# lijingzhu1/SKGHOI

Hardware: AMD Instinct MI355X
Metric: images/sec through interaction head (20x20 pairs) (higher is better)
Workload: dtype f32; 1 GPU; HICO-DET-shaped synthetic cached detections: 20 humans x 20 objects per image (G=800 grid rows, P=780 pairs, K=117 verbs), eval forward of InteractionHead from cached AdaMixer-R50 box features [40,256,7,7]/image; precision=fp32, batch_per_gpu=256, parallelism=dp1 (independent image shards, no data-path collective)

## Files before the change

### skghoi_amd/csrc/skg_gemm.hip

```cpp
#include "skg_common.h"
#include <string.h>
#include <atomic>
#include <type_traits>

__device__ __forceinline__ float skg_exp2i(int e) { return __uint_as_float((uint32_t)(127 + e) << 23); }

typedef _Float16 f16x8 __attribute__((ext_vector_type(8)));
typedef _Float16 h16x2 __attribute__((ext_vector_type(2)));
typedef uint32_t u32x4 __attribute__((ext_vector_type(4)));
typedef short s16x8 __attribute__((ext_vector_type(8)));
typedef __bf16 bf16x2_t __attribute__((ext_vector_type(2)));
typedef float f32x2_t __attribute__((ext_vector_type(2)));

__device__ __forceinline__ uint32_t skg_pack_bf16x2(float a, float b) {
    const f32x2_t v = {a, b};
    return __builtin_bit_cast(uint32_t, __builtin_convertvector(v, bf16x2_t));
}
__device__ __forceinline__ void skg_store_bf16x4(uint16_t* p, float a, float b, float c, float e) {
    *reinterpret_cast<uint2*>(p) = make_uint2(skg_pack_bf16x2(a, b), skg_pack_bf16x2(c, e));
}
__device__ __forceinline__ void skg_store_bf16(uint16_t* p, float a) { *p = (uint16_t)(skg_pack_bf16x2(a, 0.f) & 0xffffu); }

#define BM 128
#define BN 128
// ... 1048 lines not shown
struct skg_gemm_group_args {
    skg_gemm_desc d[SKG_GEMM_GROUP_MAX];
    int start[SKG_GEMM_GROUP_MAX + 1];
    int n;
};

__global__ __launch_bounds__(256, SKG_MINW) void skg_gemm_group_kernel(const skg_gemm_group_args g) {
    __shared__ __attribute__((aligned(16))) float smem[2 * (A_TILE + B_TILE)];
    int k = 0;
#pragma unroll
    for (int t = 1; t < SKG_GEMM_GROUP_MAX; ++t)
        if (t < g.n && (int)blockIdx.x >= g.start[t]) k = t;
    skg_gemm_tile<-1, 0, 2>(g.d[k], blockIdx.x - g.start[k], smem);
}

__global__ __launch_bounds__(256, SKG_MINW) void skg_gemm_group_split_kernel(const skg_gemm_group_args g) {
    __shared__ __attribute__((aligned(16))) float smem[2 * (A_TILE + B_TILE)];
    int k = 0;
#pragma unroll
    for (int t = 1; t < SKG_GEMM_GROUP_MAX; ++t)
        if (t < g.n && (int)blockIdx.x >= g.start[t]) k = t;
    skg_gemm_tile<-1, 2, 2>(g.d[k], blockIdx.x - g.start[k], smem);
}

__global__ __launch_bounds__(256, SKG_MINW) void skg_gemm_group_small_kernel(const skg_gemm_group_args g) {
    __shared__ __attribute__((aligned(16))) float smem[4 * 32 * 36];
    int k = 0;
#pragma unroll
    for (int t = 1; t < SKG_GEMM_GROUP_MAX; ++t)
        if (t < g.n && (int)blockIdx.x >= g.start[t]) k = t;
    skg_gemm_tile<-1, 1, 1>(g.d[k], blockIdx.x - g.start[k], smem);
}

__global__ __launch_bounds__(256, SKG_NB4 > 2 ? 1 : SKG_MINW) void skg_gemm_group_direct_kernel(const skg_gemm_group_args g) {
    __shared__ __attribute__((aligned(1024))) float smem[SKG_SMEM4];
    int k = 0;
#pragma unroll
    for (int t = 1; t < SKG_GEMM_GROUP_MAX; ++t)
        if (t < g.n && (int)blockIdx.x >= g.start[t]) k = t;
    skg_gemm_tile<-1, 4, 1>(g.d[k], blockIdx.x - g.start[k], smem);
}

__global__ __launch_bounds__(256, SKG_MINW) void skg_gemm_group_latency_kernel(const skg_gemm_group_args g) {
    __shared__ __attribute__((aligned(16))) float smem[SKG_SMEM3];
    int k = 0;
#pragma unroll
    for (int t = 1; t < SKG_GEMM_GROUP_MAX; ++t)
        if (t < g.n && (int)blockIdx.x >= g.start[t]) k = t;
    skg_gemm_tile<-1, 3, 1>(g.d[k], blockIdx.x - g.start[k], smem);
}

__global__ __launch_bounds__(512, 1) void skg_gemm_group_khalves_kernel(const skg_gemm_group_args g) {
    __shared__ __attribute__((aligned(16))) float smem[SKG_SMEM3];
    int k = 0;
#pragma unroll
    for (int t = 1; t < SKG_GEMM_GROUP_MAX; ++t)
        if (t < g.n && (int)blockIdx.x >= g.start[t]) k = t;
    skg_gemm_tile<-1, 5, 1>(g.d[k], blockIdx.x - g.start[k], smem);
}

#define SKG_SMEM6(T) (2 * 2 * 64 * (T) * 32)
template <int EPI, int T>
__global__ __launch_bounds__(256, 2) void skg_gemm_b16_kernel(const skg_gemm_desc d, const uint16_t* w16) {
    __shared__ __attribute__((aligned(1024))) float smem[SKG_SMEM6(T)];
    skg_gemm_tile<EPI, 6, T>(d, blockIdx.x, smem, w16);
}
// ... 107 lines not shown
    const int src = a_rows ? a_rows[row] : row;
    uint32_t mx = 0u;
    if (src >= 0) {
        const float* p = A + (int64_t)src * lda;
        for (int k = 4 * lane; k < K; k += 256) {
            const float4 v = *reinterpret_cast<const float4*>(p + k);
            mx = max(max(mx, __float_as_uint(v.x) & 0x7fffffffu), __float_as_uint(v.y) & 0x7fffffffu);
            mx = max(max(mx, __float_as_uint(v.z) & 0x7fffffffu), __float_as_uint(v.w) & 0x7fffffffu);
        }
    }
#pragma unroll
    for (int off = 32; off > 0; off >>= 1) mx = max(mx, (uint32_t)__shfl_xor((int)mx, off, 64));
    if (lane == 0) {
        const int E = (int)(mx >> 23);
        exp_out[row] = (mx == 0u || E == 255) ? 0 : min(max(E - 127 - 11, -126), 126);
    }
}

extern "C" int skg_row_exponents_f32(const float* A, int64_t lda, const int32_t* a_rows, int M, int K, int32_t* exp_out,
                                     void* stream) {
    if (M < 0 || K <= 0 || (K & 3) || (lda & 3)) return SKG_E_ARG;
    if (M == 0) return 0;
    if (!A || !exp_out) return SKG_E_ARG;
    if (!skg_aligned16(A)) return SKG_E_ALIGN;
    hipLaunchKernelGGL(skg_row_exponents_kernel, dim3((M + 3) / 4), dim3(256), 0, (hipStream_t)stream, A, lda, a_rows, M, K,
                       exp_out);
    return skg_launch_status();
}

#define g_small_mode skg_tune_small_mode()
#define g_khalves_blocks skg_tune_khalves_blocks()
#define g_small_tiles skg_tune_small_tiles()

static int skg_gemm_tile_scale(const skg_gemm_desc* d) {
    const bool glds = SKG_USE_GLDS && BK == 16 && (d->K % BK) == 0 && !d->a_rows &&
                      (int64_t)BM * d->lda * 4 < 0xffffffffLL && (int64_t)BN * d->ldw * 4 < 0xffffffffLL;
    const int64_t tiles128 = (int64_t)((d->M + 127) / 128) * ((d->N + 127) / 128) * (d->split_k > 1 ? d->split_k : 1);
    if (d->w_split && (d->K % 16) == 0 && d->w_scale > 0.f) return 2;
    return (glds && (tiles128 < g_small_tiles || d->M <= 64)) ? 1 : 2;
}

extern "C" int skg_gemm_dot_partials(const skg_gemm_desc* dh) {
    if (!dh) return SKG_E_ARG;
    const int T = skg_gemm_tile_scale(dh);
    return 2 * ((dh->N + 64 * T - 1) / (64 * T));
}

static int skg_gemm_validate(const skg_gemm_desc& d) {
    if (d.split_k > 1 && (!d.split_ws || (d.epilogue != SKG_EPI_BIAS && d.epilogue != SKG_EPI_BIAS_RELU &&
                                          d.epilogue != SKG_EPI_BIAS_RES_RELU) || d.split_k > 64))
        return SKG_E_ARG;
    if (d.M < 0 || d.N <= 0 || d.K <= 0 || !d.A || !d.W) return SKG_E_ARG;
    if ((d.K & 3) || (d.lda & 3) || (d.ldw & 3)) return SKG_E_ALIGN;
    if (!skg_aligned16(d.A) || !skg_aligned16(d.W)) return SKG_E_ALIGN;
    if (d.lda < d.K && !d.a_rows && d.M > 1) return SKG_E_ARG;
    switch (d.epilogue) {
        case SKG_EPI_BIAS: case SKG_EPI_BIAS_RELU:
            if (!d.C) return SKG_E_ARG; break;
        case SKG_EPI_MUL_RELU:
            if (!d.C || (!d.P && !d.Q)) return SKG_E_ARG; break;
        case SKG_EPI_RELU_DOT:
            if (!d.dot_w || !d.dot_partial) return SKG_E_ARG; break;
        case SKG_EPI_BIAS_RES_RELU:
            if (!d.C || !d.res) return SKG_E_ARG; break;
        default: return SKG_E_ARG;
    }
    return 0;
}

#define g_route_tiles skg_tune_route_tiles()

static bool skg_route_desc(const skg_gemm_desc& d, skg_gemmx_desc& x, skg_gemmx_fused& f) {
    if (d.w_split || d.a_rows || d.a_exp || d.epilogue == SKG_EPI_RELU_DOT) return false;
    memset(&x, 0, sizeof(x)); memset(&f, 0, sizeof(f));
    x.A = d.A; x.a_sm = d.lda; x.a_sk = 1;
    x.B = d.W; x.b_sn = d.ldw; x.b_sk = 1;
    x.C = d.C; x.ldc = d.ldc; x.M = d.M; x.N = d.N; x.K = d.K;
    x.bias = d.bias; x.relu = d.epilogue == SKG_EPI_BIAS_RELU ? 1 : 0;
    x.split_k = d.split_k > 1 ? d.split_k : 0; x.split_ws = d.split_ws;
    f.out_rows = d.out_rows;
    if (d.epilogue == SKG_EPI_MUL_RELU) {
        f.kind = SKG_EPI_MUL_RELU;
        f.P = d.P; f.p_idx = d.p_idx; f.ldp = d.ldp; f.Q = d.Q; f.q_idx = d.q_idx; f.ldq = d.ldq; f.mbias = d.mbias;
        f.C_raw = d.C_raw; f.ldc_raw = d.ldc_raw;
    } else if (d.epilogue == SKG_EPI_BIAS_RES_RELU) {
        f.kind = SKG_EPI_BIAS_RES_RELU; f.res = d.res; f.ldres = d.ldres;
    }
    return skg_gemmx_can_fuse(&x, &f) != 0;
}

static bool skg_gemm_group_small(const skg_gemm_desc* descs, int n) {
    int64_t tiles128 = 0;
    for (int i = 0; i < n; ++i) {
        const skg_gemm_desc& d = descs[i];
        if (d.M == 0) continue;
        const bool glds = SKG_USE_GLDS && BK == 16 && (d.K % BK) == 0 && !d.a_rows &&
                          (int64_t)BM * d.lda * 4 < 0xffffffffLL && (int64_t)BN * d.ldw * 4 < 0xffffffffLL;
        if (!glds || (d.w_split && d.w_scale > 0.f)) return false;
        tiles128 += (int64_t)((d.M + 127) / 128) * ((d.N + 127) / 128);
    }
    return tiles128 < g_small_tiles;
}

static std::atomic<long long> g_gemm_path[SKG_GEMM_PATHS];
static inline void skg_gemm_count(int path) { g_gemm_path[path].fetch_add(1, std::memory_order_relaxed); }

extern "C" void skg_gemm_path_counts(int64_t* out_host, int reset) {
    for (int i = 0; i < SKG_GEMM_PATHS; ++i) {
        if (out_host) out_host[i] = g_gemm_path[i].load(std::memory_order_relaxed);
        if (reset) g_gemm_path[i].store(0, std::memory_order_relaxed);
    }
}

extern "C" int skg_gemm_group_tile(const skg_gemm_desc* descs_host, int n) {
    if (!descs_host || n < 1 || n > SKG_GEMM_GROUP_MAX) return SKG_E_ARG;
    return skg_gemm_group_small(descs_host, n) ? 1 : 2;
}

extern "C" int skg_gemm_group_f32(const skg_gemm_desc* descs_host, int n, void* stream) {
    if (!descs_host || n < 1 || n > SKG_GEMM_GROUP_MAX) return SKG_E_ARG;
    skg_gemm_group_args g, r;
    g.n = r.n = 0;
    int64_t blocks = 0, rblocks = 0;
    bool split = true;
    for (int i = 0; i < n; ++i) {
        const int rc = skg_gemm_validate(descs_host[i]);
        if (rc) return rc;
    }
    const bool small = skg_gemm_group_small(descs_host, n);
    if (n <= SKG_GEMMX_GROUP_MAX) {
// ... 4 lines not shown
        for (int i = 0; i < n && ok; ++i) {
            const skg_gemm_desc& d = descs_host[i];
            ok = skg_route_desc(d, xs[i], fs[i]);
            tiles128 += (int64_t)((d.M + 127) / 128) * ((d.N + 127) / 128) * (d.split_k > 1 ? d.split_k : 1);
        }
        if (ok && tiles128 >= g_route_tiles && tiles128 < 4 * g_small_tiles) {
            skg_gemm_count(SKG_GEMM_PATH_ROUTED);
            return skg_gemmx_f32_fused(xs, fs, n, stream);
        }
    }
    for (int i = 0; i < n; ++i) {
        const skg_gemm_desc& d = descs_host[i];
        if (d.split_k > 1 && !small) return SKG_E_ARG;
        if (d.M == 0) continue;
        split = split && d.w_split && (d.K % 16) == 0 && d.w_scale > 0.f;
        const int64_t nb = skg_gemm_blocks(d.M, d.N, d.K, small ? 1 : 2) * (d.split_k > 1 ? d.split_k : 1);
        if (blocks + nb > 0x7fffffffLL) return SKG_E_LIMIT;
        g.d[g.n] = d;
        g.start[g.n] = (int)blocks;
        blocks += nb;
        ++g.n;
        if (d.split_k > 1) {
            r.d[r.n] = d;
            r.start[r.n] = (int)rblocks;
            rblocks += ((int64_t)d.M * d.N + 255) / 256;
            ++r.n;
        }
    }
    if (g.n == 0) return 0;
    for (int i = g.n; i <= SKG_GEMM_GROUP_MAX; ++i) g.start[i] = (int)blocks;
    bool direct = small && g_small_mode == 4;
    for (int i = 0; i < g.n && direct; ++i) direct = (g.d[i].K % 64) == 0;
    const bool halves = small && (g_small_mode == 5 || (g_small_mode == 6 && blocks <= g_khalves_blocks));
    skg_gemm_count(split && !small ? SKG_GEMM_PATH_FP16X2 : SKG_GEMM_PATH_EXACT);
    if (direct) hipLaunchKernelGGL(skg_gemm_group_direct_kernel, dim3((unsigned)blocks), dim3(256), 0, (hipStream_t)stream, g);
    else if (halves) hipLaunchKernelGGL(skg_gemm_group_khalves_kernel, dim3((unsigned)blocks), dim3(512), 0, (hipStream_t)stream, g);
    else if (small && g_small_mode >= 3) hipLaunchKernelGGL(skg_gemm_group_latency_kernel, dim3((unsigned)blocks), dim3(256), 0, (hipStream_t)stream, g);
    else if (small) hipLaunchKernelGGL(skg_gemm_group_small_kernel, dim3((unsigned)blocks), dim3(256), 0, (hipStream_t)stream, g);
    else if (split) hipLaunchKernelGGL(skg_gemm_group_split_kernel, dim3((unsigned)blocks), dim3(256), 0, (hipStream_t)stream, g);
    else hipLaunchKernelGGL(skg_gemm_group_kernel, dim3((unsigned)blocks), dim3(256), 0, (hipStream_t)stream, g);
    if (r.n) {
        for (int i = r.n; i <= SKG_GEMM_GROUP_MAX; ++i) r.start[i] = (int)rblocks;
        hipLaunchKernelGGL(skg_splitk_reduce_group_kernel, dim3((unsigned)rblocks), dim3(256), 0, (hipStream_t)stream, r);
    }
    return skg_launch_status();
}

extern "C" int skg_gemm_f32(const skg_gemm_desc* dh, void* stream) {
    if (!dh) return SKG_E_ARG;
    const skg_gemm_desc d = *dh;
    const int rc = skg_gemm_validate(d);
    if (rc) return rc;
    if (d.M == 0) return 0;
    const bool glds = SKG_USE_GLDS && BK == 16 && (d.K % BK) == 0 && !d.a_rows &&
                      (int64_t)BM * d.lda * 4 < 0xffffffffLL && (int64_t)BN * d.ldw * 4 < 0xffffffffLL;
    const bool split = d.w_split && (d.K % 16) == 0 && d.w_scale > 0.f;
    const int T = split ? 2 : skg_gemm_tile_scale(&d);
    if (!split && T == 1 && d.M > 64) {
        const int64_t tiles128 = (int64_t)((d.M + 127) / 128) * ((d.N + 127) / 128) * (d.split_k > 1 ? d.split_k : 1);
        skg_gemmx_desc x; skg_gemmx_fused f;
        if (tiles128 >= g_route_tiles && skg_route_desc(d, x, f)) {
            skg_gemm_count(SKG_GEMM_PATH_ROUTED);
            return skg_gemmx_f32_fused(&x, &f, 1, stream);
        }
    }
    const int64_t nblk = skg_gemm_blocks(d.M, d.N, d.K, T) * (d.split_k > 1 ? d.split_k : 1);
    if (nblk > 0x7fffffffLL) return SKG_E_LIMIT;
    dim3 grid((unsigned)nblk), block(256);
    hipStream_t s = (hipStream_t)stream;
    skg_gemm_count(split ? SKG_GEMM_PATH_FP16X2 : SKG_GEMM_PATH_EXACT);
#define SKG_LAUNCH(E)                                                                              \
    if (split) hipLaunchKernelGGL((skg_gemm_kernel<E, 2, 2>), grid, block, 0, s, d);               \
    else if (glds && T == 1 && g_small_mode == 4 && (d.K % 64) == 0) hipLaunchKernelGGL((skg_gemm_kernel<E, 4, 1>), grid, block, 0, s, d); \
    else if (glds && T == 1 && (g_small_mode == 5 || (g_small_mode == 6 && nblk <= g_khalves_blocks))) hipLaunchKernelGGL((skg_gemm_kernel<E, 5, 1>), grid, dim3(512), 0, s, d); \
    else if (glds && T == 1 && g_small_mode >= 3) hipLaunchKernelGGL((skg_gemm_kernel<E, 3, 1>), grid, block, 0, s, d); \
    else if (glds && T == 1) hipLaunchKernelGGL((skg_gemm_kernel<E, 1, 1>), grid, block, 0, s, d); \
    else if (glds) hipLaunchKernelGGL((skg_gemm_kernel<E, 1, 2>), grid, block, 0, s, d);           \
    else hipLaunchKernelGGL((skg_gemm_kernel<E, 0, 2>), grid, block, 0, s, d);
    switch (d.epilogue) {
        case SKG_EPI_BIAS:          SKG_LAUNCH(SKG_EPI_BIAS) break;
        case SKG_EPI_BIAS_RELU:     SKG_LAUNCH(SKG_EPI_BIAS_RELU) break;
        case SKG_EPI_MUL_RELU:      SKG_LAUNCH(SKG_EPI_MUL_RELU) break;
        case SKG_EPI_RELU_DOT:      SKG_LAUNCH(SKG_EPI_RELU_DOT) break;
        case SKG_EPI_BIAS_RES_RELU: SKG_LAUNCH(SKG_EPI_BIAS_RES_RELU) break;
    }
#undef SKG_LAUNCH
    if (d.split_k > 1) {
        const int64_t total = (int64_t)d.M * d.N;
// ... 302 lines not shown
```

### skghoi_amd/csrc/skg_pairs.hip

```cpp
#include "skg_common.h"

#define PS_THREADS 256
__global__ __launch_bounds__(PS_THREADS) void skg_pairs_spatial_kernel(
    const float* __restrict__ boxes, const skg_image_meta* __restrict__ meta, int32_t* __restrict__ grid_h,
    int32_t* __restrict__ grid_o, int32_t* __restrict__ grid_pair, int32_t* __restrict__ grid_img,
    int32_t* __restrict__ pair_grid, int64_t* __restrict__ x_keep, int64_t* __restrict__ y_keep,
    int32_t* __restrict__ pair_h, int32_t* __restrict__ pair_o, float* __restrict__ spatial, int scrub_nan,
    int grid_cap, int pair_cap) {
    __shared__ float4 sbox[SKG_MAX_NODES];
    const int a = blockIdx.x;
    const skg_image_meta mt = meta[a];
    const int lane = threadIdx.x;
    const int n = mt.n, n_h = mt.n_h;
    for (int t = lane; t < n; t += PS_THREADS)
        sbox[t] = *reinterpret_cast<const float4*>(boxes + 4 * (int64_t)(mt.box_off + t));
    __syncthreads();

    const float h = mt.img_h, w = mt.img_w;
    const float eps = 1e-10f;
    const int G = n_h * n;
    bool any_nan = false;
    for (int r = lane; r < G; r += PS_THREADS) {
        const int i = r / n, j = r - i * n;
        const int gr = mt.grid_off + r;
// ... 138 lines not shown
    const int t = threadIdx.x;
    const float4 v = reinterpret_cast<const float4*>(src)[t];
    if (out) reinterpret_cast<float4*>(dst)[t] = v;
    if (out16) skg_store_twin4(out16 + (int64_t)r * out_ld + 4 * t, v);
    if (t < 64) {
        const float* e = ent + ((int64_t)ent_img[r] * SKG_TRANSH_ENT + ent_row[r]) * SKG_TRANSH_DIM;
        const float x = (t < SKG_TRANSH_DIM) ? e[t] : 0.f;
        if (out) dst[1024 + t] = x;
        if (out16) out16[(int64_t)r * out_ld + 1024 + t] = (uint16_t)skg_pack_bf16(x, 0.f);
    }
}

extern "C" int skg_concat_entity_x(const float* enc, int64_t ld_enc, const int32_t* enc_row, const float* ent,
                                   const int32_t* ent_img, const int32_t* ent_row, int rows, void* out, int64_t out_ld,
                                   int out_dtype, void* stream) {
    if (rows < 0 || (out_dtype != SKG_DTYPE_F32 && out_dtype != SKG_DTYPE_BF16)) return SKG_E_ARG;
    if (rows == 0) return 0;
    if (!enc || !enc_row || !ent || !ent_img || !ent_row || !out || out_ld < 1088) return SKG_E_ARG;
    const bool half = out_dtype == SKG_DTYPE_BF16;
    if (!skg_aligned16(enc) || (half ? (((uintptr_t)out) & 7u) != 0 : !skg_aligned16(out)) || (ld_enc & 3) || (out_ld & 3))
        return SKG_E_ALIGN;
    float* o32 = half ? nullptr : (float*)out;
    hipLaunchKernelGGL(skg_concat_entity_kernel, dim3(rows), dim3(256), 0, (hipStream_t)stream, enc, ld_enc, enc_row,
                       ent, ent_img, ent_row, o32, out_ld, half ? (uint16_t*)out : skg_twin(o32));
    return skg_launch_status();
}

extern "C" int skg_concat_entity_f32(const float* enc, int64_t ld_enc, const int32_t* enc_row, const float* ent,
                                     const int32_t* ent_img, const int32_t* ent_row, int rows, float* out,
                                     int64_t out_ld, void* stream) {
    return skg_concat_entity_x(enc, ld_enc, enc_row, ent, ent_img, ent_row, rows, out, out_ld, SKG_DTYPE_F32, stream);
}

__device__ __forceinline__ void skg_rows_mul_relu_row(const skg_rows_mul_args& a, int r) {
    const float* p = a.P + (int64_t)(a.p_idx ? a.p_idx[r] : r) * a.ldp;
    const float* q = a.Q ? a.Q + (int64_t)(a.q_idx ? a.q_idx[r] : r) * a.ldq : nullptr;
    const float* f = a.F + (int64_t)(a.f_idx ? a.f_idx[r] : r) * a.ldf;
    float* o = a.out ? a.out + (int64_t)r * a.ldo : nullptr;
    uint16_t* o16 = a.out16 ? a.out16 + (int64_t)r * a.ldo : nullptr;
    for (int c = threadIdx.x * 4; c < a.cols; c += 1024) {
        float4 m = *reinterpret_cast<const float4*>(p + c);
        if (q) {
            const float4 t = *reinterpret_cast<const float4*>(q + c);
            m.x += t.x; m.y += t.y; m.z += t.z; m.w += t.w;
        }
        if (a.mbias) {
            const float4 t = *reinterpret_cast<const float4*>(a.mbias + c);
            m.x += t.x; m.y += t.y; m.z += t.z; m.w += t.w;
        }
        const float4 v = *reinterpret_cast<const float4*>(f + c);
        const float4 res = make_float4(skg_relu(m.x * v.x), skg_relu(m.y * v.y), skg_relu(m.z * v.z), skg_relu(m.w * v.w));
        if (o) *reinterpret_cast<float4*>(o + c) = res;
        if (o16) skg_store_twin4(o16 + c, res);
    }
}

struct skg_rows_mul_pack { skg_rows_mul_args a[SKG_MULTI_MAX]; };
__global__ __launch_bounds__(256) void skg_rows_mul_relu_multi_kernel(const skg_rows_mul_pack pk) {
    const skg_rows_mul_args a = pk.a[blockIdx.y];
    if ((int)blockIdx.x >= a.rows) return;
    skg_rows_mul_relu_row(a, (int)blockIdx.x);
}

static int skg_rows_mul_relu_check(skg_rows_mul_args& a, uintptr_t out_align) {
    if (a.rows < 0 || a.cols <= 0 || (a.cols & 3)) return SKG_E_ARG;
    if (a.rows == 0) return 0;
    const void* out = out_align == 8 ? (const void*)a.out16 : (const void*)a.out;
    if (!a.P || !a.F || !out) return SKG_E_ARG;
    if ((a.ldp & 3) || (a.ldf & 3) || (a.ldo & 3) || (a.Q && (a.ldq & 3))) return SKG_E_ALIGN;
    if (!skg_aligned16(a.P) || !skg_aligned16(a.F) || (((uintptr_t)out) & (out_align - 1)) || !skg_aligned16(a.Q) ||
        !skg_aligned16(a.mbias))
        return SKG_E_ALIGN;
    if (out_align != 8) a.out16 = skg_twin(a.out);
    return 0;
}

static int skg_rows_mul_relu_launch(const skg_rows_mul_args* calls, int n, uintptr_t out_align, void* stream) {
    if (!calls || n < 1 || n > SKG_MULTI_MAX) return SKG_E_ARG;
    skg_rows_mul_pack pk;
    int m = 0, rows = 0;
    for (int i = 0; i < n; ++i) {
        pk.a[m] = calls[i];
        if (const int e = skg_rows_mul_relu_check(pk.a[m], out_align)) return e;
        if (pk.a[m].rows == 0) continue;
        rows = pk.a[m].rows > rows ? pk.a[m].rows : rows;
        ++m;
    }
    if (m == 0) return 0;
    hipLaunchKernelGGL(skg_rows_mul_relu_multi_kernel, dim3(rows, m), dim3(256), 0, (hipStream_t)stream, pk);
    return skg_launch_status();
}

int skg_rows_mul_relu_multi(const skg_rows_mul_args* calls, int n, void* stream) {
    return skg_rows_mul_relu_launch(calls, n, 16, stream);
}

extern "C" int skg_rows_mul_relu_x(const float* P, const int32_t* p_idx, int64_t ldp, const float* Q,
                                   const int32_t* q_idx, int64_t ldq, const float* mbias, const float* F,
                                   const int32_t* f_idx, int64_t ldf, int rows, int cols, void* out, int64_t ldo,
                                   int out_dtype, void* stream) {
    if (out_dtype != SKG_DTYPE_F32 && out_dtype != SKG_DTYPE_BF16) return SKG_E_ARG;
    const bool half = out_dtype == SKG_DTYPE_BF16;
    const skg_rows_mul_args a = {P, p_idx, ldp, Q, q_idx, ldq, mbias, F, f_idx, ldf, rows, cols,
                                 half ? nullptr : (float*)out, ldo, half ? (uint16_t*)out : nullptr};
    return skg_rows_mul_relu_launch(&a, 1, half ? 8 : 16, stream);
}

extern "C" int skg_rows_mul_relu_f32(const float* P, const int32_t* p_idx, int64_t ldp, const float* Q,
                                     const int32_t* q_idx, int64_t ldq, const float* mbias, const float* F,
                                     const int32_t* f_idx, int64_t ldf, int rows, int cols, float* out, int64_t ldo,
                                     void* stream) {
    return skg_rows_mul_relu_x(P, p_idx, ldp, Q, q_idx, ldq, mbias, F, f_idx, ldf, rows, cols, out, ldo, SKG_DTYPE_F32,
                               stream);
}

__global__ __launch_bounds__(256) void skg_transpose_kernel(const float* __restrict__ in, int64_t ld_in, int rows,
                                                            int cols, float* __restrict__ out, int64_t ld_out) {
    __shared__ float tile[64][65];
    const int r0 = blockIdx.y * 64, c0 = blockIdx.x * 64;
    const int tx = threadIdx.x & 63, ty = threadIdx.x >> 6;
    for (int i = ty; i < 64; i += 4) {
        const int r = r0 + i, c = c0 + tx;
// ... 19 lines not shown
```

### skghoi_amd/engine.py

```python
import ctypes as C
import os
import threading

import numpy as np
import torch

from . import _capi, layout, transh

EPS_LN = 1e-5

GEMM_TIMER = None
GEMM_TIMER_EPI = None

import os as _os
_PIN_TABLES = _os.environ.get("SKG_PIN_TABLES", "1") == "1"
_NO_SPIN = _os.environ.get("SKG_NO_SPIN", "0") == "1"


_SHARED_STREAMS = {}


def shared_side_stream(dev, priority=0, slot=0):
    dev = torch.device(dev)
    key = (dev.index if dev.index is not None else torch.cuda.current_device(), priority, slot)
# ... 545 lines not shown

    def get(self, i):
        if self.thread is None:
            while self.drawn <= i:
                self._draw(self.drawn)
                self.drawn += 1
            return self.out[i]
        self.ready[i].wait()
        if self.err is not None:
            raise self.err
        return self.out[i]

    def release(self, i, event):
        self.events[i] = event
        self.slots[i % len(self.slots)]["event"] = event
        self.released[i].set()

    def join(self):
        self.abort = True
        for ev in self.released:
            ev.set()
        if self.thread is not None:
            self.thread.join()
        if self.err is not None and not isinstance(self.err, _DrawAborted):
            raise self.err


class Preprocessed:
    pass


class HeadEngine:
    GROUP_FC2_BELOW = 32768

    def __init__(self, graph_head, predictor, suppressor, human_idx, num_classes, box_nms_thresh, box_score_thresh,
                 max_human, max_object, faithful_skip_offset=True):
        self.gh = graph_head
        self.predictor = predictor
        self.suppressor = suppressor
        self.human_idx = int(human_idx)
        self.K = int(num_classes)
        self.box_nms_thresh = float(box_nms_thresh)
        self.box_score_thresh = float(box_score_thresh)
        self.max_human = int(max_human)
        self.max_object = int(max_object)
        self.faithful_skip_offset = faithful_skip_offset
        self.chunk_images = 128
        self.debug = False
        self.transh_device = None
        self._slots = None
        self._streams = None
        self.n_streams = 2
        self.precision = "fp32"
        self.inference_precision = None
        self.inference_activations = None
        self._pw = None
        self._vt = None
        self._det_off_cache = {}
        self._gt_const = None
        self._cnt_host = None
        self._cnt_event = None
        self._cnt_host_dev = None
        self.plan_epoch = 0
        self._ck_events = None
        self.small_two_branches = os.environ.get("SKG_SMALL_ONE_BRANCH") != "1"
        self.g1_on_side_branch = os.environ.get("SKG_G1_ON_SIDE", "0") == "1"
# ... 288 lines not shown
        Mp = lay.sum_p
        meta_g = torch.from_numpy(lay.meta.view(np.int32).reshape(-1).copy()).to(dev, non_blocking=True)
        x_keep = torch.empty(max(Mp, 1), device=dev, dtype=torch.int64); y_keep = torch.empty_like(x_keep)
        PF = torch.empty(max(Mp, 1), 2048, **f32)
        sc = torch.empty(max(Mp, 1), self.K, **f32) if want_scores else None
        keep = {} if self.debug else None
        tabs = []
        step = max(int(self.chunk_images), 1)
        bounds = [(a0, min(A, a0 + step)) for a0 in range(0, A, step)]
        drawer = None
        on_device = tables is None and self.transh_device is not None
        if tables is None and not on_device:
            drawer = _TableDrawer(self.K, [b - a for a, b in bounds], want_scores,
                                  self._table_slots(max(b - a for a, b in bounds), want_scores))
        try:
            lookahead = 2
            ctxs = {}

            main = torch.cuda.current_stream()
            ns = max(1, int(self.n_streams)) if len(bounds) > 1 else 1
            if ns > 1:
                if self._streams is None or len(self._streams) < ns:
                    self._streams = [shared_side_stream(dev, 0, slot=i) for i in range(ns)]
                ev0 = torch.cuda.Event(); ev0.record(main)
                for st_ in self._streams[:ns]:
                    st_.wait_event(ev0)

            def on_stream(ci):
                return torch.cuda.stream(self._streams[ci % ns]) if ns > 1 else _NullCtx()

            def phase_a(ci):
                a0, a1 = bounds[ci]
                with on_stream(ci):
                    ctxs[ci] = self._chunk_phase_a(layout.chunk(lay, a0, a1), pw, pre, G1, x_keep, y_keep, PF, a16=a16)

            for ci in range(min(lookahead, len(bounds))):
                phase_a(ci)
            for ci, (a0, a1) in enumerate(bounds):
                if on_device:
                    with on_stream(ci):
                        t = transh.device_tables(pre.boxes, pre.scores, pre.labels, ctxs[ci]["meta"], a1 - a0, self.K,
                                                 want_scores, *self.transh_device)
                elif tables is None:
                    t = drawer.get(ci)
                else:
                    t = tuple(None if x is None else x[a0:a1] for x in tables)
                with on_stream(ci):
                    if self.debug:
                        tabs.append(tuple(None if x is None else x.clone() for x in t))
                    self._chunk_phase_b(ctxs.pop(ci), t, pw, pre, enc, PF, sc, keep)
                    if drawer is not None:
                        ev = torch.cuda.Event(); ev.record(current_stream_of(None))
                        drawer.release(ci, ev)
                if ci + lookahead < len(bounds):
                    phase_a(ci + lookahead)
            if ns > 1:
                for st_ in self._streams[:ns]:
                    ev = torch.cuda.Event(); ev.record(st_)
                    main.wait_event(ev)
        finally:
            if drawer is not None:
                drawer.join()
        out.update(x_keep=x_keep[:Mp], y_keep=y_keep[:Mp], meta=meta_g, pair_features=PF[:Mp])
        if tabs:
            out["tables"] = tuple(None if tabs[0][i] is None else torch.cat([t[i] for t in tabs]) for i in range(3))
        if want_scores:
            out["transh_scores"] = sc[:Mp]
        if keep is not None:
            for k, v in keep.items():
                out[k] = torch.cat(v)
        return out

    def _chunk_phase_a(self, ch, pw, pre, G1, x_keep, y_keep, PF, ibuf=None, offs=None, meta=None, caps=None, a16=False):
        lib = _capi.lib()
        dev = pre.device
        st = _stream()
        f32 = dict(device=dev, dtype=torch.float32)
        i32 = dict(device=dev, dtype=torch.int32)
        A = ch.n_active
        Mh, Mn, Mg, Mp = ch.sum_h, ch.sum_n, ch.sum_g, ch.sum_p
        if ibuf is None:
            buf, offs = layout.pack_int_arrays(ch)
            ibuf = torch.from_numpy(buf).to(dev, non_blocking=True)

        def isl(name):
            o, l = offs[name]
            return ibuf[o:o + l]

        if meta is None:
            meta = isl("meta")
        xk = x_keep[ch.P0:]; yk = y_keep[ch.P0:]
        grid_h = torch.empty(Mg, **i32); grid_o = torch.empty(Mg, **i32); grid_pair = torch.empty(Mg, **i32)
        grid_img = torch.empty(Mg, **i32); pair_grid = torch.empty(max(Mp, 1), **i32)
        pair_h = torch.empty(max(Mp, 1), **i32); pair_o = torch.empty(max(Mp, 1), **i32)
        sp48 = torch.empty(Mg, _capi.SPATIAL_LD, **f32)
        gcap, pcap = caps if caps is not None else (0, 0)
        _capi.check(lib.skg_pairs_spatial_padded_f32(pre.boxes.data_ptr(), meta.data_ptr(), A, grid_h.data_ptr(),
                                                     grid_o.data_ptr(), grid_pair.data_ptr(), grid_img.data_ptr(),
                                                     pair_grid.data_ptr(), xk.data_ptr(), yk.data_ptr(),
                                                     pair_h.data_ptr(), pair_o.data_ptr(), sp48.data_ptr(), 1, gcap, pcap,
                                                     st), "skg_pairs_spatial_padded_f32")
        s1 = torch.empty(Mg, 128, device=dev, dtype=self._adt(a16, 128))
        s2 = torch.empty(Mg, 256, device=dev, dtype=self._adt(a16, 256))
        S = torch.empty(Mg, 1024, device=dev, dtype=self._adt(a16, 1024))
        gemm(sp48, pw.sp0_w, pw.sp0_b, s1, Mg, 128, _capi.SPATIAL_LD, _capi.EPI_BIAS_RELU)
        gemm(s1, pw.sp2_w, pw.sp2_b, s2, Mg, 256, 128, _capi.EPI_BIAS_RELU)
        gemm(s2, pw.sp4_w, pw.sp4_b, S, Mg, 1024, 256, _capi.EPI_BIAS_RELU)
        del s1, s2
        cx = dict(ch=ch, isl=isl, meta=meta, grid_h=grid_h, grid_o=grid_o, grid_img=grid_img, grid_pair=grid_pair,
                  pair_grid=pair_grid, pair_h=pair_h, pair_o=pair_o, sp48=sp48, S=S, ibuf=ibuf, a16=a16)
        if G1 is not None:
            self._chunk_phase_a2(cx, pw, pre, G1, PF)
        return cx

    def _chunk_phase_a2(self, cx, pw, pre, G1, PF):
        ch = cx["ch"]
        Mg, Mp = ch.sum_g, ch.sum_p
        Tg = torch.empty(max(Mp, 1), 1024, device=pre.device, dtype=self._adt(cx.get("a16", False), 1024))
        if Mp:
            gemm(cx["S"], pw.att_g["w2"], pw.att_g["b2"], Tg, Mg, 1024, 1024, _capi.EPI_MUL_RELU, P=G1,
                 p_idx=cx["grid_img"], ldp=1024, out_rows=cx["grid_pair"])
            gemm(Tg, pw.att_g["w3"], pw.att_g["b3"], PF, Mp, 1024, 1024, _capi.EPI_BIAS_RELU, ldc=2048,
                 C_off=ch.P0 * 2048 + 1024)
        cx["Tg"] = Tg

    def _chunk_phase_b(self, cx, tabs, pw, pre, enc, PF, sc, keep, need_S=None, need_Tg=None):
        lib = _capi.lib()
        gh = self.gh
        dev = pre.device
        st = _stream()
        f32 = dict(device=dev, dtype=torch.float32)
        ch, isl, meta = cx["ch"], cx["isl"], cx["meta"]
        grid_h, grid_o, pair_grid, pair_h, pair_o = cx["grid_h"], cx["grid_o"], cx["pair_grid"], cx["pair_h"], cx["pair_o"]
        sp48, S = cx["sp48"], cx["S"]
        A = ch.n_active
        Mh, Mn, Mg, Mp = ch.sum_h, ch.sum_n, ch.sum_g, ch.sum_p
        ent, rel, nrm = tabs
        ent_d = ent.to(dev, non_blocking=True)
        a16 = cx.get("a16", False)
        adt = self._adt(a16, 1024)
        odt = _capi.DTYPE_BF16 if adt == torch.bfloat16 else _capi.DTYPE_F32
        a16 = adt == torch.bfloat16
        F2 = torch.empty(Mg, 1024, **f32)
        if gh.num_iter > 0:
            X = torch.empty(Mh + Mn, 1088, device=dev, dtype=adt)
            rows, eimg, erow = isl("enc_row_hn"), isl("img_hn"), isl("ent_row_hn")
            if a16:
                _capi.check(lib.skg_concat_entity_x(enc.data_ptr(), 1024, rows.data_ptr(), ent_d.data_ptr(),
                                                    eimg.data_ptr(), erow.data_ptr(), Mh + Mn, X.data_ptr(), 1088, odt, st),
                            "skg_concat_entity_x")
            else:
                _capi.check(lib.skg_concat_entity_f32(enc.data_ptr(), 1024, rows.data_ptr(), ent_d.data_ptr(),
                                                      eimg.data_ptr(), erow.data_ptr(), Mh + Mn, X.data_ptr(), 1088, st),
                            "skg_concat_entity_f32")
            GH = torch.empty(Mh, 1024, **f32); GO = torch.empty(Mn, 1024, **f32)
            GHa = torch.empty(Mh, 1024, device=dev, dtype=adt) if a16 else GH
            GOa = torch.empty(Mn, 1024, device=dev, dtype=adt) if a16 else GO
# ... 41 lines not shown
                                                        Tos.data_ptr(), Tso.data_ptr(), 1024, 1024, U.data_ptr(),
                                                        V.data_ptr(), 1024, adj.data_ptr(), st),
                            "skg_graph_aggregate_f32")
            del T, Tos, Tso
            Hp = torch.empty(Mh, 1024, **f32); Op = torch.empty(Mn, 1024, **f32)
            gemm_group([((U, pw.os["w3"], pw.os["b3"], Hp, Mh, 1024, 1024, _capi.EPI_BIAS_RES_RELU),
                         dict(res=GH, ldres=1024)),
                        ((V, pw.so["w3"], pw.so["b3"], Op, Mn, 1024, 1024, _capi.EPI_BIAS_RES_RELU),
                         dict(res=GO, ldres=1024))])
            h_node = torch.empty(Mh, 1024, device=dev, dtype=adt); node = torch.empty(Mn, 1024, device=dev, dtype=adt)
            if a16:
                _capi.check(lib.skg_layernorm2_x(Hp.data_ptr(), 1024, pw.nh_g.data_ptr(), pw.nh_b.data_ptr(), Mh,
                                                 h_node.data_ptr(), 1024, Op.data_ptr(), 1024, pw.no_g.data_ptr(),
                                                 pw.no_b.data_ptr(), Mn, node.data_ptr(), 1024, 1024, EPS_LN, odt, st),
                            "skg_layernorm2_x")
            else:
                _capi.check(lib.skg_layernorm2_f32(Hp.data_ptr(), 1024, pw.nh_g.data_ptr(), pw.nh_b.data_ptr(), Mh,
                                                   h_node.data_ptr(), 1024, Op.data_ptr(), 1024, pw.no_g.data_ptr(),
                                                   pw.no_b.data_ptr(), Mn, node.data_ptr(), 1024, 1024, EPS_LN, st),
                            "skg_layernorm2_f32")
        else:
            if need_S is not None:
                need_S()
            gemm(S, pw.att["w2"], pw.att["b2"], F2, Mg, 1024, 1024, _capi.EPI_BIAS)
            h_node = enc.index_select(0, isl("hum_enc_row").long())
            node = enc.index_select(0, isl("node_enc_row").long())
            adj = None
        if Mp:
            B1h = torch.empty(Mh, 1024, **f32); B1o = torch.empty(Mn, 1024, **f32)
            gemm_group([((h_node, pw.att["w1"], None, B1h, Mh, 1024, 1024, _capi.EPI_BIAS), dict(ldw=2048)),
                        ((node, pw.att["w1"], None, B1o, Mn, 1024, 1024, _capi.EPI_BIAS), dict(ldw=2048, W_off=1024))])
            if need_Tg is not None:
                need_Tg()
            Tp = cx["Tg"]
            if Tp.dtype == torch.bfloat16:
                _capi.check(lib.skg_rows_mul_relu_x(B1h.data_ptr(), pair_h.data_ptr(), 1024, B1o.data_ptr(),
                                                    pair_o.data_ptr(), 1024, pw.att["b1"].data_ptr(), F2.data_ptr(),
                                                    pair_grid.data_ptr(), 1024, Mp, 1024, Tp.data_ptr(), 1024,
                                                    _capi.DTYPE_BF16, st), "skg_rows_mul_relu_x")
            else:
                _capi.check(lib.skg_rows_mul_relu_f32(B1h.data_ptr(), pair_h.data_ptr(), 1024, B1o.data_ptr(),
                                                      pair_o.data_ptr(), 1024, pw.att["b1"].data_ptr(), F2.data_ptr(),
                                                      pair_grid.data_ptr(), 1024, Mp, 1024, Tp.data_ptr(), 1024, st),
                            "skg_rows_mul_relu_f32")
            gemm(Tp, pw.att["w3"], pw.att["b3"], PF, Mp, 1024, 1024, _capi.EPI_BIAS_RELU, ldc=2048,
                 C_off=ch.P0 * 2048)
        if sc is not None:
            rel_d = rel.to(dev, non_blocking=True); nrm_d = nrm.to(dev, non_blocking=True)
            _capi.check(lib.skg_transh_scores_f32(ent_d.data_ptr(), rel_d.data_ptr(), nrm_d.data_ptr(), self.K,
                                                  self.human_idx, meta.data_ptr(), A,
                                                  sc.data_ptr() + 4 * ch.P0 * self.K, st), "skg_transh_scores_f32")
        if keep is not None:
            keep.setdefault("spatial46", []).append(sp48)
            keep.setdefault("h_node", []).append(h_node); keep.setdefault("node", []).append(node)
            if adj is not None:
                keep.setdefault("adjacency", []).append(adj)

    def _classify(self, pair_features, pw):
        dev = pair_features.device
        Mp = pair_features.shape[0]
        ld = (self.K + 1 + 3) // 4 * 4
        logits = torch.empty(max(Mp, 1), ld, device=dev, dtype=torch.float32)
        if pw.fused_cls:
            if Mp:
                sk = pick_split_k(Mp, self.K + 1, 2048)
                ws = torch.empty(sk, Mp, self.K + 1, device=dev, dtype=torch.float32) if sk > 1 else None
                gemm(pair_features, pw.cls_w, pw.cls_b, logits, Mp, self.K + 1, 2048, _capi.EPI_BIAS, split_k=sk,
                     split_ws=ws)
        else:
            logits[:Mp, :self.K] = self.predictor(pair_features)
            logits[:Mp, self.K:self.K + 1] = self.suppressor(pair_features)
        return logits[:Mp]

    def score(self, logits, pre, g, training, out=None, L_dev=None):
        lib = _capi.lib()
        lay = g["layout"]
        dev = pre.device
        vt = self.verbs(dev)
        Mp, Lt = lay.sum_p, lay.sum_l
# ... 18 lines not shown
```

Before: 8676 images/s.

## Group paired fc3 GEMMs into one launch and batch rows in mul-relu kernel

```diff
diff --git a/skghoi_amd/csrc/skg_gemm.hip b/skghoi_amd/csrc/skg_gemm.hip
--- a/skghoi_amd/csrc/skg_gemm.hip
+++ b/skghoi_amd/csrc/skg_gemm.hip
@@ -1104,6 +1104,16 @@
     skg_gemm_tile<-1, 1, 1>(g.d[k], blockIdx.x - g.start[k], smem);
 }
 
+template <int EPI>
+__global__ __launch_bounds__(256, SKG_MINW) void skg_gemm_group_dma_kernel(const skg_gemm_group_args g) {
+    __shared__ __attribute__((aligned(1024))) float smem[2 * (A_TILE + B_TILE)];
+    int k = 0;
+#pragma unroll
+    for (int t = 1; t < SKG_GEMM_GROUP_MAX; ++t)
+        if (t < g.n && (int)blockIdx.x >= g.start[t]) k = t;
+    skg_gemm_tile<EPI, 1, 2>(g.d[k], blockIdx.x - g.start[k], smem);
+}
+
 __global__ __launch_bounds__(256, SKG_NB4 > 2 ? 1 : SKG_MINW) void skg_gemm_group_direct_kernel(const skg_gemm_group_args g) {
     __shared__ __attribute__((aligned(1024))) float smem[SKG_SMEM4];
     int k = 0;
@@ -1277,9 +1287,13 @@
 #define g_khalves_blocks skg_tune_khalves_blocks()
 #define g_small_tiles skg_tune_small_tiles()
 
+static bool skg_gemm_glds_ok(const skg_gemm_desc& d) {
+    return SKG_USE_GLDS && BK == 16 && (d.K % BK) == 0 && !d.a_rows &&
+           (int64_t)BM * d.lda * 4 < 0xffffffffLL && (int64_t)BN * d.ldw * 4 < 0xffffffffLL;
+}
+
 static int skg_gemm_tile_scale(const skg_gemm_desc* d) {
-    const bool glds = SKG_USE_GLDS && BK == 16 && (d->K % BK) == 0 && !d->a_rows &&
-                      (int64_t)BM * d->lda * 4 < 0xffffffffLL && (int64_t)BN * d->ldw * 4 < 0xffffffffLL;
+    const bool glds = skg_gemm_glds_ok(*d);
     const int64_t tiles128 = (int64_t)((d->M + 127) / 128) * ((d->N + 127) / 128) * (d->split_k > 1 ? d->split_k : 1);
     if (d->w_split && (d->K % 16) == 0 && d->w_scale > 0.f) return 2;
     return (glds && (tiles128 < g_small_tiles || d->M <= 64)) ? 1 : 2;
@@ -1339,8 +1353,7 @@
     for (int i = 0; i < n; ++i) {
         const skg_gemm_desc& d = descs[i];
         if (d.M == 0) continue;
-        const bool glds = SKG_USE_GLDS && BK == 16 && (d.K % BK) == 0 && !d.a_rows &&
-                          (int64_t)BM * d.lda * 4 < 0xffffffffLL && (int64_t)BN * d.ldw * 4 < 0xffffffffLL;
+        const bool glds = skg_gemm_glds_ok(d);
         if (!glds || (d.w_split && d.w_scale > 0.f)) return false;
         tiles128 += (int64_t)((d.M + 127) / 128) * ((d.N + 127) / 128);
     }
@@ -1411,6 +1424,26 @@
     bool direct = small && g_small_mode == 4;
     for (int i = 0; i < g.n && direct; ++i) direct = (g.d[i].K % 64) == 0;
     const bool halves = small && (g_small_mode == 5 || (g_small_mode == 6 && blocks <= g_khalves_blocks));
+    bool dma = !small;
+    int64_t dma_tiles = 0;
+    for (int i = 0; i < g.n && dma; ++i) {
+        const skg_gemm_desc& d = g.d[i];
+        dma = d.epilogue == g.d[0].epilogue && skg_gemm_glds_ok(d) && !d.w_split && d.split_k <= 1;
+        dma_tiles += (int64_t)((d.M + 127) / 128) * ((d.N + 127) / 128);
+    }
+    if (dma && dma_tiles >= 4 * (int64_t)g_small_tiles) {
+        const dim3 grid((unsigned)blocks), block(256);
+        hipStream_t s = (hipStream_t)stream;
+        skg_gemm_count(SKG_GEMM_PATH_EXACT);
+        switch (g.d[0].epilogue) {
+            case SKG_EPI_BIAS:          hipLaunchKernelGGL(skg_gemm_group_dma_kernel<SKG_EPI_BIAS>, grid, block, 0, s, g); break;
+            case SKG_EPI_BIAS_RELU:     hipLaunchKernelGGL(skg_gemm_group_dma_kernel<SKG_EPI_BIAS_RELU>, grid, block, 0, s, g); break;
+            case SKG_EPI_MUL_RELU:      hipLaunchKernelGGL(skg_gemm_group_dma_kernel<SKG_EPI_MUL_RELU>, grid, block, 0, s, g); break;
+            case SKG_EPI_RELU_DOT:      hipLaunchKernelGGL(skg_gemm_group_dma_kernel<SKG_EPI_RELU_DOT>, grid, block, 0, s, g); break;
+            case SKG_EPI_BIAS_RES_RELU: hipLaunchKernelGGL(skg_gemm_group_dma_kernel<SKG_EPI_BIAS_RES_RELU>, grid, block, 0, s, g); break;
+        }
+        return skg_launch_status();
+    }
     skg_gemm_count(split && !small ? SKG_GEMM_PATH_FP16X2 : SKG_GEMM_PATH_EXACT);
     if (direct) hipLaunchKernelGGL(skg_gemm_group_direct_kernel, dim3((unsigned)blocks), dim3(256), 0, (hipStream_t)stream, g);
     else if (halves) hipLaunchKernelGGL(skg_gemm_group_khalves_kernel, dim3((unsigned)blocks), dim3(512), 0, (hipStream_t)stream, g);
@@ -1431,8 +1464,7 @@
     const int rc = skg_gemm_validate(d);
     if (rc) return rc;
     if (d.M == 0) return 0;
-    const bool glds = SKG_USE_GLDS && BK == 16 && (d.K % BK) == 0 && !d.a_rows &&
-                      (int64_t)BM * d.lda * 4 < 0xffffffffLL && (int64_t)BN * d.ldw * 4 < 0xffffffffLL;
+    const bool glds = skg_gemm_glds_ok(d);
     const bool split = d.w_split && (d.K % 16) == 0 && d.w_scale > 0.f;
     const int T = split ? 2 : skg_gemm_tile_scale(&d);
     if (!split && T == 1 && d.M > 64) {
diff --git a/skghoi_amd/csrc/skg_pairs.hip b/skghoi_amd/csrc/skg_pairs.hip
--- a/skghoi_amd/csrc/skg_pairs.hip
+++ b/skghoi_amd/csrc/skg_pairs.hip
@@ -194,34 +194,54 @@
     return skg_concat_entity_x(enc, ld_enc, enc_row, ent, ent_img, ent_row, rows, out, out_ld, SKG_DTYPE_F32, stream);
 }
 
-__device__ __forceinline__ void skg_rows_mul_relu_row(const skg_rows_mul_args& a, int r) {
-    const float* p = a.P + (int64_t)(a.p_idx ? a.p_idx[r] : r) * a.ldp;
-    const float* q = a.Q ? a.Q + (int64_t)(a.q_idx ? a.q_idx[r] : r) * a.ldq : nullptr;
-    const float* f = a.F + (int64_t)(a.f_idx ? a.f_idx[r] : r) * a.ldf;
-    float* o = a.out ? a.out + (int64_t)r * a.ldo : nullptr;
-    uint16_t* o16 = a.out16 ? a.out16 + (int64_t)r * a.ldo : nullptr;
+constexpr int SKG_ROWS_MUL_R = 4;
+__device__ __forceinline__ void skg_rows_mul_relu_rows(const skg_rows_mul_args& a, int r0) {
+    constexpr int R = SKG_ROWS_MUL_R;
+    const int last = a.rows - 1;
+    const float* p[R]; const float* q[R]; const float* f[R];
+#pragma unroll
+    for (int j = 0; j < R; ++j) {
+        const int r = r0 + j < last ? r0 + j : last;
+        p[j] = a.P + (int64_t)(a.p_idx ? a.p_idx[r] : r) * a.ldp;
+        q[j] = a.Q ? a.Q + (int64_t)(a.q_idx ? a.q_idx[r] : r) * a.ldq : nullptr;
+        f[j] = a.F + (int64_t)(a.f_idx ? a.f_idx[r] : r) * a.ldf;
+    }
     for (int c = threadIdx.x * 4; c < a.cols; c += 1024) {
-        float4 m = *reinterpret_cast<const float4*>(p + c);
-        if (q) {
-            const float4 t = *reinterpret_cast<const float4*>(q + c);
-            m.x += t.x; m.y += t.y; m.z += t.z; m.w += t.w;
-        }
-        if (a.mbias) {
-            const float4 t = *reinterpret_cast<const float4*>(a.mbias + c);
-            m.x += t.x; m.y += t.y; m.z += t.z; m.w += t.w;
-        }
-        const float4 v = *reinterpret_cast<const float4*>(f + c);
-        const float4 res = make_float4(skg_relu(m.x * v.x), skg_relu(m.y * v.y), skg_relu(m.z * v.z), skg_relu(m.w * v.w));
-        if (o) *reinterpret_cast<float4*>(o + c) = res;
-        if (o16) skg_store_twin4(o16 + c, res);
+        float4 pv[R], qv[R], fv[R];
+#pragma unroll
+        for (int j = 0; j < R; ++j) {
+            if (j > 0 && p[j] == p[j - 1]) pv[j] = pv[j - 1];
+            else pv[j] = *reinterpret_cast<const float4*>(p[j] + c);
+            if (q[j]) {
+                if (j > 0 && q[j] == q[j - 1]) qv[j] = qv[j - 1];
+                else qv[j] = *reinterpret_cast<const float4*>(q[j] + c);
+            }
+            if (j > 0 && f[j] == f[j - 1]) fv[j] = fv[j - 1];
+            else fv[j] = *reinterpret_cast<const float4*>(f[j] + c);
+        }
+        float4 mb = make_float4(0.f, 0.f, 0.f, 0.f);
+        if (a.mbias) mb = *reinterpret_cast<const float4*>(a.mbias + c);
+#pragma unroll
+        for (int j = 0; j < R; ++j) {
+            if (r0 + j > last) break;
+            float4 m = pv[j];
+            if (q[j]) { m.x += qv[j].x; m.y += qv[j].y; m.z += qv[j].z; m.w += qv[j].w; }
+            if (a.mbias) { m.x += mb.x; m.y += mb.y; m.z += mb.z; m.w += mb.w; }
+            const float4 v = fv[j];
+            const float4 res = make_float4(skg_relu(m.x * v.x), skg_relu(m.y * v.y), skg_relu(m.z * v.z), skg_relu(m.w * v.w));
+            const int64_t o = (int64_t)(r0 + j) * a.ldo + c;
+            if (a.out) *reinterpret_cast<float4*>(a.out + o) = res;
+            if (a.out16) skg_store_twin4(a.out16 + o, res);
+        }
     }
 }
 
 struct skg_rows_mul_pack { skg_rows_mul_args a[SKG_MULTI_MAX]; };
 __global__ __launch_bounds__(256) void skg_rows_mul_relu_multi_kernel(const skg_rows_mul_pack pk) {
     const skg_rows_mul_args a = pk.a[blockIdx.y];
-    if ((int)blockIdx.x >= a.rows) return;
-    skg_rows_mul_relu_row(a, (int)blockIdx.x);
+    const int r0 = (int)blockIdx.x * SKG_ROWS_MUL_R;
+    if (r0 >= a.rows) return;
+    skg_rows_mul_relu_rows(a, r0);
 }
 
 static int skg_rows_mul_relu_check(skg_rows_mul_args& a, uintptr_t out_align) {
@@ -249,7 +269,7 @@
         ++m;
     }
     if (m == 0) return 0;
-    hipLaunchKernelGGL(skg_rows_mul_relu_multi_kernel, dim3(rows, m), dim3(256), 0, (hipStream_t)stream, pk);
+    hipLaunchKernelGGL(skg_rows_mul_relu_multi_kernel, dim3((rows + SKG_ROWS_MUL_R - 1) / SKG_ROWS_MUL_R, m), dim3(256), 0, (hipStream_t)stream, pk);
     return skg_launch_status();
 }
 
diff --git a/skghoi_amd/engine.py b/skghoi_amd/engine.py
--- a/skghoi_amd/engine.py
+++ b/skghoi_amd/engine.py
@@ -601,6 +601,7 @@
 
 class HeadEngine:
     GROUP_FC2_BELOW = 32768
+    PAIR_FC3_FROM = 32768
 
     def __init__(self, graph_head, predictor, suppressor, human_idx, num_classes, box_nms_thresh, box_score_thresh,
                  max_human, max_object, faithful_skip_offset=True):
@@ -955,7 +956,8 @@
             def phase_a(ci):
                 a0, a1 = bounds[ci]
                 with on_stream(ci):
-                    ctxs[ci] = self._chunk_phase_a(layout.chunk(lay, a0, a1), pw, pre, G1, x_keep, y_keep, PF, a16=a16)
+                    ctxs[ci] = self._chunk_phase_a(layout.chunk(lay, a0, a1), pw, pre, G1, x_keep, y_keep, PF, a16=a16,
+                                                   pair_fc3=True)
 
             for ci in range(min(lookahead, len(bounds))):
                 phase_a(ci)
@@ -994,7 +996,8 @@
                 out[k] = torch.cat(v)
         return out
 
-    def _chunk_phase_a(self, ch, pw, pre, G1, x_keep, y_keep, PF, ibuf=None, offs=None, meta=None, caps=None, a16=False):
+    def _chunk_phase_a(self, ch, pw, pre, G1, x_keep, y_keep, PF, ibuf=None, offs=None, meta=None, caps=None, a16=False,
+                       pair_fc3=False):
         lib = _capi.lib()
         dev = pre.device
         st = _stream()
@@ -1032,6 +1035,8 @@
         del s1, s2
         cx = dict(ch=ch, isl=isl, meta=meta, grid_h=grid_h, grid_o=grid_o, grid_img=grid_img, grid_pair=grid_pair,
                   pair_grid=pair_grid, pair_h=pair_h, pair_o=pair_o, sp48=sp48, S=S, ibuf=ibuf, a16=a16)
+        cx["pair_fc3"] = bool(pair_fc3 and Mp >= self.PAIR_FC3_FROM and not a16 and _active_splits() is None
+                              and _active_bf16() is None)
         if G1 is not None:
             self._chunk_phase_a2(cx, pw, pre, G1, PF)
         return cx
@@ -1043,9 +1048,15 @@
         if Mp:
             gemm(cx["S"], pw.att_g["w2"], pw.att_g["b2"], Tg, Mg, 1024, 1024, _capi.EPI_MUL_RELU, P=G1,
                  p_idx=cx["grid_img"], ldp=1024, out_rows=cx["grid_pair"])
-            gemm(Tg, pw.att_g["w3"], pw.att_g["b3"], PF, Mp, 1024, 1024, _capi.EPI_BIAS_RELU, ldc=2048,
-                 C_off=ch.P0 * 2048 + 1024)
+            if not cx.get("pair_fc3"):
+                a, kw = self._global_fc3(Tg, pw, PF, ch)
+                gemm(*a, **kw)
         cx["Tg"] = Tg
+
+    @staticmethod
+    def _global_fc3(Tg, pw, PF, ch):
+        return ((Tg, pw.att_g["w3"], pw.att_g["b3"], PF, ch.sum_p, 1024, 1024, _capi.EPI_BIAS_RELU),
+                dict(ldc=2048, C_off=ch.P0 * 2048 + 1024))
 
     def _chunk_phase_b(self, cx, tabs, pw, pre, enc, PF, sc, keep, need_S=None, need_Tg=None):
         lib = _capi.lib()
@@ -1153,7 +1164,8 @@
                         ((node, pw.att["w1"], None, B1o, Mn, 1024, 1024, _capi.EPI_BIAS), dict(ldw=2048, W_off=1024))])
             if need_Tg is not None:
                 need_Tg()
-            Tp = cx["Tg"]
+            paired = cx.get("pair_fc3", False)
+            Tp = torch.empty_like(cx["Tg"]) if paired else cx["Tg"]
             if Tp.dtype == torch.bfloat16:
                 _capi.check(lib.skg_rows_mul_relu_x(B1h.data_ptr(), pair_h.data_ptr(), 1024, B1o.data_ptr(),
                                                     pair_o.data_ptr(), 1024, pw.att["b1"].data_ptr(), F2.data_ptr(),
@@ -1164,8 +1176,12 @@
                                                       pair_o.data_ptr(), 1024, pw.att["b1"].data_ptr(), F2.data_ptr(),
                                                       pair_grid.data_ptr(), 1024, Mp, 1024, Tp.data_ptr(), 1024, st),
                             "skg_rows_mul_relu_f32")
-            gemm(Tp, pw.att["w3"], pw.att["b3"], PF, Mp, 1024, 1024, _capi.EPI_BIAS_RELU, ldc=2048,
-                 C_off=ch.P0 * 2048)
+            fc3 = ((Tp, pw.att["w3"], pw.att["b3"], PF, Mp, 1024, 1024, _capi.EPI_BIAS_RELU),
+                   dict(ldc=2048, C_off=ch.P0 * 2048))
+            if paired:
+                gemm_group([fc3, self._global_fc3(cx["Tg"], pw, PF, ch)])
+            else:
+                gemm(*fc3[0], **fc3[1])
         if sc is not None:
             rel_d = rel.to(dev, non_blocking=True); nrm_d = nrm.to(dev, non_blocking=True)
             _capi.check(lib.skg_transh_scores_f32(ent_d.data_ptr(), rel_d.data_ptr(), nrm_d.data_ptr(), self.K,
```

Measured after the change: 8656 images/s. No clear change (-0.2%).
